# SketchyScene/SketchySceneColorization

Hardware: AMD Instinct MI355X
Metric: train images/sec (192x192, gen+disc fwd+bwd) (higher is better)
Workload: dtype fp32 (bf16x6 split on the bf16 MFMA, fp32 accumulate; filter gradients and few-channel layers on the exact-fp32 MFMA); 1 GPU; Foreground_Instance_Colorization Pix2Pix GAN train step (D-step + G-step, TF-Adam), 192x192, batch 32 per GPU; global_batch=32, parallelism=dp1, ranks_observed_by_allreduce=1, launcher=in-process, block_type=Pix2Pix, launch=hipGraph replay

## Files before the change

### include/sketchycolor_hip.h

```cpp
#ifndef SKETCHYCOLOR_HIP_H
#define SKETCHYCOLOR_HIP_H

#include <stdint.h>

#ifdef __cplusplus
extern "C" {
#endif

#define SSC_ACT_NONE 0
#define SSC_ACT_RELU 1
#define SSC_ACT_LRELU 2
#define SSC_ACT_TANH 3
#define SSC_ACT_PRELU 5
#define SSC_ACT_MIU 4

typedef struct ssc_gview {
    const float* s0;
    const float* s1;
    const float* ab0;
    const float* ab1;
    int32_t C0, C1;
    int32_t H, W;
    int32_t act;
    int32_t act1;
// ... 80 lines not shown
int ssc_conv_forward_bn(const ssc_conv_desc* d, float* ws, int64_t ws_bytes, const float* scale, const float* offset,
                        float eps, float* ab, float* stats, void* stream);
int ssc_head1_forward_supported(const ssc_conv_desc* d);
int ssc_head1_forward(const ssc_conv_desc* d, float* ws, int64_t ws_bytes, void* stream);
int ssc_head1_dgrad_supported(const ssc_conv_desc* d);
int ssc_head1_dgrad(const ssc_conv_desc* d, void* stream);
int ssc_head1_wgrad_supported(const ssc_wgrad_desc* d);
int ssc_head1_wgrad(const ssc_wgrad_desc* d, float* ws, int64_t ws_bytes, void* stream);
int ssc_head1_dgrad_bn_backward(const ssc_conv_desc* d, const float* x, const float* ab, const float* stats, int act,
                                const float* rowb, float rowb_scale, float* dx, float* dscale, float* doffset, float* ws,
                                int64_t ws_bytes, void* stream);
int ssc_bn_bwd_finalize(const float* partial, int nblk, int C, int64_t M, float* coef, float* dscale, float* doffset,
                        void* stream);
int ssc_conv_narrow_supported(const ssc_conv_desc* d);
int ssc_conv_narrow_forward(const ssc_conv_desc* d, void* stream);
int ssc_conv_pw1x1_supported(const ssc_conv_desc* d);
int ssc_conv_c3x3_supported(const ssc_conv_desc* d);
int ssc_conv_s2n16_supported(const ssc_conv_desc* d);
int ssc_conv_tr4n16_supported(const ssc_conv_desc* d);
int ssc_conv_fewchan7_supported(const ssc_conv_desc* d);
int ssc_conv_tr4_tiny_supported(const ssc_conv_desc* d);
int ssc_conv_fewchan_supported(const ssc_conv_desc* d);
int ssc_conv_forward_kernel_name(const ssc_conv_desc* d, char* buf, int len);
int ssc_conv_wgrad_kernel_name(const ssc_wgrad_desc* d, char* buf, int len);
int ssc_conv_forward_plan(const ssc_conv_desc* d, int64_t ws_bytes, int* out5);
int ssc_conv_wgrad_plan(const ssc_wgrad_desc* d, int64_t ws_bytes, int* out4);
int ssc_conv_wgrad128_plan(const ssc_wgrad_desc* d, int64_t ws_bytes, int* out7);
int ssc_conv_bf_plan(const ssc_conv_desc* d, int64_t ws_bytes, int* out10);

int ssc_nchw_to_nhwc(const float* src, float* dst, int N, int C, int HW, int ldc, int coff, void* stream);
// ... 229 lines not shown
```

### sketchyscenecolorization_amd/build.py

```python
import os
import subprocess
import sys

HERE = os.path.dirname(os.path.abspath(__file__))
ROOT = os.path.dirname(HERE)
CSRC = os.path.join(HERE, 'csrc')
LIB_DIR = os.path.join(HERE, 'lib')
LIB_PATH = os.path.join(LIB_DIR, 'libsketchycolor_hip.so')
EXTRA_FLAGS = {'igemm.hip': ['-Xclang', '-target-feature', '-Xclang', '-load-store-opt']} if os.environ.get('SSC_NO_LSOPT') == '1' else {}
NO_PACKED_FP32 = {'narrow.hip': []}
VGPR_FORM = ['-mllvm', '-amdgpu-mfma-vgpr-form=1']
LAST_BUILD = None
SOURCES = ['igemm.hip', 'igemm_bf16.hip', 'wgrad128.hip', 'wgrad128_bf16.hip', 'wgn16.hip', 'narrow.hip', 'head1.hip', 'fewchan.hip', 'fewchan7.hip', 'pw1x1.hip', 'c3x3.hip', 's2n16.hip', 'tr4tiny.hip', 'tr4n16.hip', 'elementwise.hip', 'text_lstm.hip', 'losses_optim.hip', 'mru_ops.hip', 'bg_io.hip', 'bg_scene.hip', 'fg_scene.hip', 'metrics.hip', 'matching.hip', 'match_eval.hip', 'match_train.hip']


def _hipcc():
    for c in (os.environ.get('HIPCC'), '/opt/rocm/bin/hipcc', 'hipcc'):
        if c and (os.path.isabs(c) and os.path.exists(c) or not os.path.isabs(c)):
            return c
    return 'hipcc'


HASH_MARKER = b'SSC_CSRC_HASH='


def tree_hash(csrc=None, header=None):
    import hashlib
    csrc = csrc or CSRC
# ... 33 lines not shown
    import hashlib
    objs = []
    procs = []
    hdrs = b''
    for hp in sorted(os.path.join(CSRC, f) for f in os.listdir(CSRC) if f.endswith('.h')) + [os.path.join(ROOT, 'include', 'sketchycolor_hip.h')]:
        with open(hp, 'rb') as fh:
            hdrs += fh.read()
    for s in SOURCES:
        src = os.path.join(CSRC, s)
        if not os.path.exists(src):
            continue
        obj = os.path.join(LIB_DIR, s.replace('.hip', '.o'))
        cmd = [_hipcc(), '--offload-arch=gfx950', '-O3', '-std=c++17', '-fPIC', '-I' + os.path.join(ROOT, 'include'),
               '-Wno-unused-value', '-Wno-unused-function'] + NO_PACKED_FP32.get(s, ['-fno-slp-vectorize']) + \
              os.environ.get('SSC_EXTRA_HIPCC_FLAGS', '').split() + \
              EXTRA_FLAGS.get(s, []) + (VGPR_FORM if s in ('igemm_bf16.hip', 'wgrad128_bf16.hip') else []) + (['-DSSC_CSRC_HASH="%s"' % th] if s == 'elementwise.hip' else []) + ['-c', src, '-o', obj]
        objs.append(obj)
        with open(src, 'rb') as fh:
            key = hashlib.sha256(fh.read() + b'\0' + hdrs + b'\0' + ' '.join(cmd).encode()).hexdigest()
        kf = obj + '.key'
        if not force and os.path.exists(obj) and os.path.exists(kf) and open(kf).read() == key:
            continue
        if verbose:
            print(' '.join(cmd), flush=True)
        procs.append((subprocess.Popen(cmd), cmd, kf, key))
    for p, cmd, kf, key in procs:
        if p.wait() != 0:
            raise RuntimeError('hipcc failed: ' + ' '.join(cmd))
        with open(kf, 'w') as fh:
            fh.write(key)
    cmd = [_hipcc(), '--offload-arch=gfx950', '-shared', '-fPIC', '-o', LIB_PATH] + objs
# ... 10 lines not shown
```

### sketchyscenecolorization_amd/csrc/igemm.hip

```cpp
#include <hip/hip_runtime.h>
#include <stdint.h>
#include <stdio.h>
#include <stdlib.h>
#include "sketchycolor_hip.h"
#include "igemm_util.h"
#include "igemm_epilogue.h"
#include "host_util.h"

extern "C" int ssc_conv_wgrad128_supported(const ssc_wgrad_desc* dp);
extern "C" int ssc_conv_wgrad128(const ssc_wgrad_desc* dp, float* ws, int64_t ws_bytes, void* stream);
int ssc_conv_wgrad128_bf_selected(const ssc_wgrad_desc* dp);
extern "C" int ssc_conv_wgn16_supported(const ssc_wgrad_desc* dp);
int ssc_conv_wgn16(const ssc_wgrad_desc* dp, float* ws, int64_t ws_bytes, void* stream);
int ssc_conv_wgn16_fits(const ssc_wgrad_desc* dp, int64_t ws_bytes);
int ssc_conv_narrow_forward_ws(const ssc_conv_desc* dp, float* ws, int64_t ws_bytes, void* stream, int* csplit_out);
int ssc_conv_fewchan_forward(const ssc_conv_desc* dp, int num_cu, void* stream);
extern "C" int ssc_conv_pw1x1_supported(const ssc_conv_desc* dp);
int ssc_conv_pw1x1_walkers(const ssc_conv_desc* dp);
int ssc_conv_pw1x1_forward(const ssc_conv_desc* dp, float* stat, void* stream);
extern "C" int ssc_conv_tr4n16_supported(const ssc_conv_desc* dp);
int ssc_conv_tr4n16_rows(const ssc_conv_desc* dp);
int ssc_conv_tr4n16_forward(const ssc_conv_desc* dp, float* stat, void* stream);
extern "C" int ssc_conv_fewchan7_supported(const ssc_conv_desc* dp);
int ssc_conv_fewchan7_walkers(const ssc_conv_desc* dp);
// ... 1457 lines not shown
            if ((double)t128 < plan_const("SSC_PLAN_BF_HK_MIN", 0.5) * 2.0 * num_cu()) {
                return plan_launch(cfgs, 5, allowed_bf, M, d.Nstore, d.nphase, nkt, (long)d.NB * d.OH * d.OW * d.ldc, ws_bytes,
                                   have_ws, can_ts, plan_const("SSC_PLAN_BF_SCALE", 0.45));
            }
            cfgs[0].res = 2;
            cfgs[0].penalty = plan_const("SSC_PLAN_BF_HK", 0.78);
            if (!fwd_is_ut(d)) cfgs[0].penalty *= (double)((d.x.C0 + 15) / 16) / (double)(2 * ((d.x.C0 + 31) / 32));
        }
        return plan_launch(cfgs, 5, allowed_bf, M, d.Nstore, d.nphase, nkt, (long)d.NB * d.OH * d.OW * d.ldc, ws_bytes,
                           have_ws, can_ts, plan_const("SSC_PLAN_BF_SCALE", 0.45));
    }
    return plan_launch(FWD_CFGS, 5, allowed, M, d.Nstore, d.nphase, nkt, (long)d.NB * d.OH * d.OW * d.ldc, ws_bytes,
                       have_ws, can_ts);
}

static void copy_name(const char* src, char* dst, int len) {
    int i = 0;
    for (; i < len - 1 && src[i]; ++i) dst[i] = src[i];
    if (len > 0) dst[i] = 0;
}

extern "C" int ssc_conv_forward_kernel_name(const ssc_conv_desc* dp, char* buf, int len) {
    if (ssc_head1_forward_supported(dp) || ssc_head1_dgrad_supported(dp)) {
        copy_name(ssc_head1_dgrad_supported(dp) ? "head1_dgrad" : "head1_fwd", buf, len);
        return 0;
    }
    if (ssc_conv_narrow_supported(dp)) {
        copy_name(dp->nphase == 4 ? "narrow_fwd<transposed>" : "narrow_fwd<conv>", buf, len);
        return 0;
    }
    if (ssc_conv_fewchan_supported(dp)) {
        copy_name(dp->x.C0 == 8 ? "conv_fewchan<8>" : "conv_fewchan<4>", buf, len);
        return 0;
    }
    if (ssc_conv_pw1x1_supported(dp)) {
        copy_name("conv_pw1x1", buf, len);
        return 0;
    }
    if (ssc_conv_c3x3_supported(dp)) {
// ... 39 lines not shown
                                   const float* offset, float eps, float* ab, float* stats, void* stream) {
    ssc_conv_desc d = *dp;
    d.stat_partial = nullptr;
    d.sb_x = nullptr;
    d.sb2_x = nullptr;
    d.stat_mode = 0;
    const long M = (long)d.NB * d.PH * d.PW;
    const long Mall = M * d.nphase;
    static int off = -1;
    if (off < 0) {
        const char* e = ssc_dev_getenv("SSC_FUSE_STATS");
        off = (e != nullptr && e[0] == '0') ? 1 : 0;
    }
    bool fused = false;
    int64_t ws_conv = ws_bytes;
    const bool earlier = ssc_head1_forward_supported(dp) || ssc_head1_dgrad_supported(dp) || ssc_conv_narrow_supported(dp) ||
                         ssc_conv_fewchan_supported(dp);
    if (!off && !earlier && ws != nullptr && d.Nstore == d.ldc &&
        (ssc_conv_pw1x1_supported(&d) || ssc_conv_c3x3_supported(&d) || ssc_conv_s2n16_supported(&d) ||
         ssc_conv_tr4_tiny_supported(&d) || ssc_conv_fewchan7_supported(&d) || ssc_conv_tr4n16_supported(&d))) {
        const int nblk = ssc_conv_pw1x1_supported(&d) ? ssc_conv_pw1x1_walkers(&d)
                         : (ssc_conv_c3x3_supported(&d) ? ssc_conv_c3x3_walkers(&d)
                            : (ssc_conv_s2n16_supported(&d) ? ssc_conv_s2n16_walkers(&d)
                               : (ssc_conv_tr4_tiny_supported(&d) ? ssc_conv_tr4_tiny_blocks(&d)
                                  : (ssc_conv_fewchan7_supported(&d) ? ssc_conv_fewchan7_walkers(&d) : ssc_conv_tr4n16_rows(&d)))));
        const int64_t need = (int64_t)nblk * 2 * d.Nstore * 4;
        if (need <= ws_bytes) {
            d.stat_partial = ws;
            const int rc = ssc_conv_forward(&d, ws, ws_bytes, stream);
            if (rc != 0) return rc;
            return ssc_bn_finalize(d.stat_partial, nblk, d.Nstore, Mall, scale, offset, eps, ab, stats, stream);
        }
    }
    const bool streaming = ssc_conv_pw1x1_supported(&d) || ssc_conv_c3x3_supported(&d) || ssc_conv_s2n16_supported(&d) ||
                           ssc_conv_tr4_tiny_supported(&d) || ssc_conv_fewchan7_supported(&d) ||
                           ssc_conv_tr4n16_supported(&d);
    if (!off && !streaming && ws != nullptr && !ssc_conv_narrow_supported(dp) && !ssc_conv_fewchan_supported(dp) && d.epi == 0 &&
        !d.accumulate && d.Nstore == d.ldc && ((d.Nstore & 3) == 0) && ((reinterpret_cast<unsigned long>(d.out) & 15) == 0) &&
        (fwd_is_ut(d) || fwd_is_utg(d) || (d.bmode == 0 && fwd_is_rowtap(d)))) {
        const Plan p = plan_fwd(d, ws_bytes, true);
        if (p.cfg >= 0 && p.splitk == 1) {
            const long mt = (M + FWD_CFGS[p.cfg].BM - 1) / FWD_CFGS[p.cfg].BM;
            const int64_t need = (int64_t)mt * d.nphase * 2 * d.Nstore * 4;
            const int64_t reserve = (need + 255) & ~(int64_t)255;
            if (reserve * 4 <= ws_bytes) {
                ws_conv = (ws_bytes - reserve) & ~(int64_t)255;
                const Plan p2 = plan_fwd(d, ws_conv, true);
                if (p2.cfg == p.cfg && p2.splitk == 1) {
                    d.stat_partial = reinterpret_cast<float*>(reinterpret_cast<char*>(ws) + ws_conv);
                    fused = true;
                    const int rc = ssc_conv_forward(&d, ws, ws_conv, stream);
                    if (rc != 0) return rc;
                    return ssc_bn_finalize(d.stat_partial, (int)(mt * d.nphase), d.Nstore, Mall, scale, offset, eps, ab, stats,
                                           stream);
                }
            }
        }
    }
    if (!off && !streaming && ws != nullptr && !ssc_conv_narrow_supported(dp) && !ssc_conv_fewchan_supported(dp) && slab_stats_ok(d) &&
        !(ssc_head1_forward_supported(dp) || ssc_head1_dgrad_supported(dp))) {
        const Plan p = plan_fwd(d, ws_bytes, true);
        if (p.cfg >= 0 && p.splitk > 1 && p.ts_s <= 1) {
            const int nblk = slab_stats_blocks(Mall, d.ldc);
            const int64_t reserve = (((int64_t)nblk * 2 * d.Nstore * 4) + 255) & ~(int64_t)255;
            ws_conv = (ws_bytes - reserve) & ~(int64_t)255;
            const Plan p2 = plan_fwd(d, ws_conv, true);
            if (ws_conv > 0 && p2.cfg == p.cfg && p2.splitk == p.splitk && p2.ts_s <= 1) {
                d.stat_partial = reinterpret_cast<float*>(reinterpret_cast<char*>(ws) + ws_conv);
                const int rc = ssc_conv_forward(&d, ws, ws_conv, stream);
                if (rc != 0) return rc;
                return ssc_bn_finalize(d.stat_partial, nblk, d.Nstore, Mall, scale, offset, eps, ab, stats, stream);
            }
            d.stat_partial = nullptr;
        }
    }
    (void)fused;
    {
        static int dbg = -1;
        if (dbg < 0) {
            const char* e = ssc_dev_getenv("SSC_DEBUG_BNPATH");
            dbg = (e != nullptr && e[0] == '1') ? 1 : 0;
        }
        if (dbg) {
            const Plan p = plan_fwd(d, ws_bytes, ws != nullptr);
            fprintf(stderr, "bnpath separate: M=%ld N=%d K=%d ut=%d utg=%d narrow=%d fewchan=%d cfg=%d splitk=%d epi=%d acc=%d\n", M * d.nphase,
                    d.Nstore, d.TH * d.TW * (d.x.C0 + d.x.C1), (int)fwd_is_ut(d), (int)fwd_is_utg(d), ssc_conv_narrow_supported(dp),
                    ssc_conv_fewchan_supported(dp), p.cfg, p.splitk, d.epi, d.accumulate);
        }
    }
    const int rc = ssc_conv_forward(&d, ws, ws_bytes, stream);
    if (rc != 0) return rc;
    return ssc_bn_stats(d.out, Mall, d.Nstore, d.ldc, scale, offset, eps, ab, stats, ws, ws_bytes, stream);
}

extern "C" int ssc_conv_forward_bnbwd(const ssc_conv_desc* dp, float* ws, int64_t ws_bytes, const float* x, int ldx,
                                      const float* ab, const float* stats, int act, float* partial, int64_t partial_bytes,
                                      int* nrows, void* stream) {
    ssc_conv_desc d = *dp;
    d.stat_partial = nullptr;
    d.sb_x = nullptr;
    d.sb2_x = nullptr;
    d.stat_mode = 0;
    *nrows = 0;
    const long M = (long)d.NB * d.PH * d.PW;
    static int off = -1;
    if (off < 0) {
        const char* e = ssc_dev_getenv("SSC_FUSE_BNBWD");
        off = (e != nullptr && e[0] == '0') ? 1 : 0;
    }
    const bool earlier = ssc_head1_forward_supported(dp) || ssc_head1_dgrad_supported(dp) || ssc_conv_narrow_supported(dp) ||
                         ssc_conv_fewchan_supported(dp);
    if (!off && !earlier && partial != nullptr && x != nullptr && ab != nullptr && stats != nullptr && d.Nstore == d.ldc &&
        (ssc_conv_c3x3_supported(&d) || ssc_conv_s2n16_supported(&d))) {
        const int nblk = ssc_conv_c3x3_supported(&d) ? ssc_conv_c3x3_walkers(&d) : ssc_conv_s2n16_walkers(&d);
        if ((int64_t)nblk * 2 * d.Nstore * 4 <= partial_bytes) {
            d.stat_partial = partial;
            d.sb_x = x; d.sb_ldx = ldx; d.sb_ab = ab; d.sb_stats = stats; d.sb_act = act;
            *nrows = nblk;
            return ssc_conv_forward(&d, ws, ws_bytes, stream);
        }
    }
    if (!off && ws != nullptr && partial != nullptr && x != nullptr && ab != nullptr && stats != nullptr &&
        !ssc_conv_c3x3_supported(&d) && !ssc_conv_s2n16_supported(&d) && !ssc_conv_narrow_supported(dp) && !ssc_conv_fewchan_supported(dp) && d.epi == 0 && !d.accumulate &&
        d.bias == nullptr && d.Nstore == d.ldc &&
        d.Nn == d.Nstore && ((d.Nstore & 3) == 0) && ((ldx & 3) == 0) && ((reinterpret_cast<unsigned long>(d.out) & 15) == 0) &&
        ((reinterpret_cast<unsigned long>(x) & 15) == 0) &&
        (fwd_is_ut(d) || fwd_is_utg(d) || (d.bmode == 0 && fwd_is_rowtap(d)))) {
        const Plan p = plan_fwd(d, ws_bytes, true);
        if (p.cfg >= 0 && p.splitk == 1) {
            const long mt = (M + FWD_CFGS[p.cfg].BM - 1) / FWD_CFGS[p.cfg].BM;
            if ((int64_t)mt * d.nphase * 2 * d.Nstore * 4 <= partial_bytes) {
                d.stat_partial = partial;
                d.sb_x = x; d.sb_ldx = ldx; d.sb_ab = ab; d.sb_stats = stats; d.sb_act = act;
                *nrows = (int)(mt * d.nphase);
            }
        }
    }
    return ssc_conv_forward(&d, ws, ws_bytes, stream);
// ... 4 lines not shown
extern "C" int ssc_minmax_finalize(const float* part, int nsplit, int N, int C, float* mnmx, void* stream);

extern "C" int ssc_conv_forward_minmax(const ssc_conv_desc* dp, float* ws, int64_t ws_bytes, float* mnmx, void* stream) {
    ssc_conv_desc d = *dp;
    d.stat_partial = nullptr;
    d.sb_x = nullptr;
    d.sb2_x = nullptr;
    d.stat_mode = 0;
    const long P = (long)d.PH * d.PW;
    const long M = (long)d.NB * P;
    static int off = -1;
    if (off < 0) {
        const char* e = ssc_dev_getenv("SSC_FUSE_MINMAX");
        off = (e != nullptr && e[0] == '0') ? 1 : 0;
    }
    if (!off && ws != nullptr && d.nphase == 1 && !ssc_conv_narrow_supported(dp) && !ssc_conv_fewchan_supported(dp) &&
        (d.epi == 0 || d.epi == 2) && !d.accumulate && d.Nstore == d.ldc && d.Nn == d.Nstore && ((d.Nstore & 3) == 0) &&
        ((reinterpret_cast<unsigned long>(d.out) & 15) == 0) && (fwd_is_ut(d) || fwd_is_utg(d))) {
        const Plan p = plan_fwd(d, ws_bytes, true);
        if (p.cfg >= 0 && p.splitk == 1 && (P % FWD_CFGS[p.cfg].BM) == 0) {
            const long mt = M / FWD_CFGS[p.cfg].BM;
            const int64_t need = (int64_t)mt * 2 * d.Nstore * 4;
            if (need * 4 <= ws_bytes) {
                const int64_t ws_conv = (ws_bytes - need) & ~(int64_t)255;
                const Plan p2 = plan_fwd(d, ws_conv, true);
                if (p2.cfg == p.cfg && p2.splitk == 1) {
                    d.stat_partial = reinterpret_cast<float*>(reinterpret_cast<char*>(ws) + ws_conv);
                    d.stat_mode = 1;
                    const int rc = ssc_conv_forward(&d, ws, ws_conv, stream);
                    if (rc != 0) return rc;
                    return ssc_minmax_finalize(d.stat_partial, (int)(P / FWD_CFGS[p.cfg].BM), d.NB, d.Nstore, mnmx, stream);
// ... 11 lines not shown
    ssc_conv_desc d = *dp;
    d.stat_partial = nullptr;
    d.sb_x = nullptr;
    d.sb2_x = nullptr;
    d.stat_mode = 0;
    *nrows = 0;
    const long M = (long)d.NB * d.PH * d.PW;
    static int off = -1;
    if (off < 0) {
        const char* e = ssc_dev_getenv("SSC_FUSE_BNBWD");
        off = (e != nullptr && e[0] == '0') ? 1 : 0;
    }
    const int C1 = d.Nstore - C0;
    if (!off && ws != nullptr && s0 != nullptr && s1 != nullptr && s0->x && s1->x && s0->ab && s1->ab && s0->stats && s1->stats &&
        s0->partial && s1->partial && C0 > 0 && C1 > 0 && (C0 % 128) == 0 && (C1 & 3) == 0 &&
        !ssc_conv_narrow_supported(dp) && !ssc_conv_fewchan_supported(dp) && d.epi == 0 && !d.accumulate &&
        d.bias == nullptr && d.Nstore == d.ldc && d.Nn == d.Nstore && ((s0->ldx | s1->ldx) & 3) == 0 &&
        ((reinterpret_cast<unsigned long>(d.out) | reinterpret_cast<unsigned long>(s0->x) |
          reinterpret_cast<unsigned long>(s1->x)) & 15) == 0 &&
        (fwd_is_ut(d) || fwd_is_utg(d))) {
        const Plan p = plan_fwd(d, ws_bytes, true);
        if (p.cfg >= 0 && p.splitk == 1 && FWD_CFGS[p.cfg].BN <= 128) {
            const long mt = (M + FWD_CFGS[p.cfg].BM - 1) / FWD_CFGS[p.cfg].BM;
            if ((int64_t)mt * d.nphase * 2 * C0 * 4 <= s0->partial_bytes && (int64_t)mt * d.nphase * 2 * C1 * 4 <= s1->partial_bytes) {
                d.stat_partial = s0->partial;
                d.sb_x = s0->x; d.sb_ldx = s0->ldx; d.sb_ab = s0->ab; d.sb_stats = s0->stats; d.sb_act = s0->act;
                d.stat_partial2 = s1->partial; d.sb2_col0 = C0;
                d.sb2_x = s1->x; d.sb2_ldx = s1->ldx; d.sb2_ab = s1->ab; d.sb2_stats = s1->stats; d.sb2_act = s1->act;
                *nrows = (int)(mt * d.nphase);
            }
        }
    }
    return ssc_conv_forward(&d, ws, ws_bytes, stream);
}

extern "C" int ssc_sk_configure(int timeout_ms, int test_withhold) {
    const unsigned long long ticks = (unsigned long long)(timeout_ms > 0 ? timeout_ms : 20000) * 100000ull;
    const unsigned cfg[4] = {(unsigned)(ticks & 0xffffffffu), (unsigned)(ticks >> 32), test_withhold ? 1u : 0u, 0u};
    const int rc = ssc_sk_configure_bf(cfg);
    if (rc != 0) return rc;
    return (int)hipMemcpyToSymbol(HIP_SYMBOL(g_sk_cfg), cfg, sizeof(cfg), 0, hipMemcpyHostToDevice);
}

extern "C" int ssc_conv_forward_plan(const ssc_conv_desc* dp, int64_t ws_bytes, int* out5) {
    if (ssc_conv_narrow_supported(dp) || ssc_conv_fewchan_supported(dp)) {
        out5[0] = -1; out5[1] = 1; out5[2] = 0; out5[3] = 1; out5[4] = 0;
        return 0;
    }
    const Plan p = plan_fwd(*dp, ws_bytes, true);
    out5[0] = p.cfg; out5[1] = p.splitk; out5[2] = (int)p.ts_full; out5[3] = p.ts_s; out5[4] = (int)(p.cost / 1000.0);
    return 0;
}

static int fwd_desc_error(const ssc_conv_desc& d) {
    if ((d.x.C0 & 3) || (d.x.C1 & 3) || d.Nstore < d.Nn || d.Nstore > d.ldc) return -1;
    if (d.nphase != 1 && d.nphase != 4) return -2;
    if (d.nphase == 4 && (d.TH != 2 || d.TW != 2 || d.KH != 4 || d.KW != 4 || d.kstep != -2 || d.out_stride != 2 ||
                          d.in_stride != 1))
        return -3;
    return 0;
}
enum { FWD_TILED = 0, FWD_HEAD1, FWD_HEAD1_DGRAD, FWD_NARROW, FWD_FEWCHAN, FWD_PW1X1, FWD_C3X3, FWD_S2N16, FWD_TR4_TINY, FWD_FEWCHAN7,
       FWD_TR4N16 };
static int fwd_early_kernel(const ssc_conv_desc* dp, bool have_ws, int64_t ws_bytes) {
    const ssc_conv_desc& d = *dp;
    if (have_ws && ssc_head1_forward_supported(dp) && (int64_t)d.NB * d.x.H * d.x.W * 16 * 4 <= ws_bytes) return FWD_HEAD1;
    if (ssc_head1_dgrad_supported(dp)) return FWD_HEAD1_DGRAD;
    if (ssc_conv_narrow_supported(dp)) return FWD_NARROW;
    if (ssc_conv_fewchan_supported(dp)) return FWD_FEWCHAN;
    if (ssc_conv_pw1x1_supported(dp)) return FWD_PW1X1;
    if (ssc_conv_c3x3_supported(dp)) return FWD_C3X3;
    if (ssc_conv_s2n16_supported(dp)) return FWD_S2N16;
    if (ssc_conv_tr4_tiny_supported(dp)) return FWD_TR4_TINY;
    if (ssc_conv_fewchan7_supported(dp)) return FWD_FEWCHAN7;
    if (ssc_conv_tr4n16_supported(dp)) return FWD_TR4N16;
    return FWD_TILED;
}
static bool fwd_bf_plain(const ssc_conv_desc& d) {
    const bool plain0 = d.x.ab0 == nullptr && d.x.act == SSC_ACT_NONE;
    const bool plain1 = d.x.C1 == 0 || (d.x.ab1 == nullptr && (d.x.act1 >= 0 ? d.x.act1 : d.x.act) == SSC_ACT_NONE);
    return plain0 && plain1;
}
// ... 5 lines not shown
    if (err != 0) return err;
    if (fwd_early_kernel(dp, have_ws, ws_bytes) != FWD_TILED || !fwd_is_bf(d)) return -10;
    const Plan p = plan_fwd(d, ws_bytes, have_ws);
    if (p.cfg < 0) return -4;
    return ssc_conv_bf_form(p.cfg, fwd_bf_plain(d), d, p.splitk, have_ws, p.ts_full, p.ts_s, ws_bytes, xcd_order(), out10);
}

extern "C" int ssc_conv_forward(const ssc_conv_desc* dp, float* ws, int64_t ws_bytes, void* stream) {
    const ssc_conv_desc& d = *dp;
    hipStream_t st = (hipStream_t)stream;
    const int err = fwd_desc_error(d);
    if (err != 0) return err;
    switch (fwd_early_kernel(dp, ws != nullptr, ws_bytes)) {
        case FWD_HEAD1: return ssc_head1_forward(dp, ws, ws_bytes, stream);
        case FWD_HEAD1_DGRAD: return ssc_head1_dgrad(dp, stream);
        case FWD_NARROW: {
            int csplit = 1;
            const int rc = ssc_conv_narrow_forward_ws(dp, ws, ws_bytes, stream, &csplit);
            if (rc != 0 || csplit == 1) return rc;
            const long out_count = (long)d.NB * d.OH * d.OW * d.ldc;
            hipLaunchKernelGGL(slab_reduce_kernel, dim3((unsigned)((out_count + 255) / 256)), dim3(256), 0, st, ws, out_count,
                               csplit, d.out, out_count, d.ldc, d.Nn, d.Nstore, d.bias, d.epi, d.accumulate);
            return (int)hipGetLastError();
        }
        case FWD_FEWCHAN: return ssc_conv_fewchan_forward(dp, num_cu(), stream);
        case FWD_PW1X1: return ssc_conv_pw1x1_forward(dp, d.stat_partial, stream);
        case FWD_C3X3: return ssc_conv_c3x3_forward(dp, d.stat_partial, stream);
        case FWD_S2N16: return ssc_conv_s2n16_forward(dp, d.stat_partial, stream);
        case FWD_TR4_TINY: return ssc_conv_tr4_tiny_forward(dp, d.stat_partial, stream);
        case FWD_FEWCHAN7: return ssc_conv_fewchan7_forward(dp, d.stat_partial, stream);
// ... 194 lines not shown
```

### sketchyscenecolorization_amd/hip.py

```python
import ctypes as C
import os

import torch

_HERE = os.path.dirname(os.path.abspath(__file__))
LIB_PATH = os.environ.get('SSC_LIB_PATH') or os.path.join(_HERE, 'lib', 'libsketchycolor_hip.so')

ACT_PRELU = 5
ACT_NONE, ACT_RELU, ACT_LRELU, ACT_TANH, ACT_MIU = 0, 1, 2, 3, 4


class GView(C.Structure):
    _fields_ = [('s0', C.c_void_p), ('s1', C.c_void_p), ('ab0', C.c_void_p), ('ab1', C.c_void_p),
                ('C0', C.c_int32), ('C1', C.c_int32), ('H', C.c_int32), ('W', C.c_int32),
                ('act', C.c_int32), ('act1', C.c_int32)]


class ConvDesc(C.Structure):
    _fields_ = [('x', GView), ('w', C.c_void_p), ('bias', C.c_void_p), ('out', C.c_void_p),
                ('NB', C.c_int32), ('PH', C.c_int32), ('PW', C.c_int32),
                ('TH', C.c_int32), ('TW', C.c_int32), ('in_stride', C.c_int32),
                ('ioff_y', C.c_int32), ('ioff_x', C.c_int32), ('nphase', C.c_int32),
                ('ky0', C.c_int32), ('kx0', C.c_int32), ('kstep', C.c_int32),
                ('KH', C.c_int32), ('KW', C.c_int32), ('wC0', C.c_int32), ('wC1', C.c_int32),
# ... 108 lines not shown
    'ssc_bn_act_backward_pre': [_P, _L, _I, _I, _P, _P, _P, _I, _I, _P, _I, _I, _I, _P, _I, _P, _P, _P, _I, _P, _F, _I, _P,
                                _L, _P],
    'ssc_head1_forward_supported': [C.POINTER(ConvDesc)],
    'ssc_head1_forward': [C.POINTER(ConvDesc), _P, _L, _P],
    'ssc_head1_dgrad_supported': [C.POINTER(ConvDesc)],
    'ssc_head1_dgrad': [C.POINTER(ConvDesc), _P],
    'ssc_head1_wgrad_supported': [C.POINTER(WgradDesc)],
    'ssc_head1_wgrad': [C.POINTER(WgradDesc), _P, _L, _P],
    'ssc_head1_dgrad_bn_backward': [C.POINTER(ConvDesc), _P, _P, _P, _I, _P, _F, _P, _P, _P, _P, _L, _P],
    'ssc_bn_bwd_finalize': [_P, _I, _I, _L, _P, _P, _P, _P],
    'ssc_block_out_backward': [_P, _P, _L, _I, _I, _P, _P, _P, _P, _P, _P, _P, _P, _P, _P, _P, _P, _P, _P, _P, _L, _P],
    'ssc_bn_bwd_sums': [C.POINTER(BnApplyJob), _P, _I, _P, _P, _P, _P, _L, _P],
    'ssc_bn_bwd_apply': [C.POINTER(BnApplyJob), _P],
    'ssc_conv_narrow_supported': [C.POINTER(ConvDesc)],
    'ssc_conv_narrow_forward': [C.POINTER(ConvDesc), _P],
    'ssc_conv_fewchan_supported': [C.POINTER(ConvDesc)],
    'ssc_conv_pw1x1_supported': [C.POINTER(ConvDesc)],
    'ssc_conv_c3x3_supported': [C.POINTER(ConvDesc)],
    'ssc_conv_s2n16_supported': [C.POINTER(ConvDesc)],
    'ssc_conv_tr4n16_supported': [C.POINTER(ConvDesc)],
    'ssc_conv_fewchan7_supported': [C.POINTER(ConvDesc)],
    'ssc_conv_tr4_tiny_supported': [C.POINTER(ConvDesc)],
    'ssc_conv_forward_kernel_name': [C.POINTER(ConvDesc), C.c_char_p, _I],
    'ssc_conv_wgrad_kernel_name': [C.POINTER(WgradDesc), C.c_char_p, _I],
    'ssc_conv_forward_plan': [C.POINTER(ConvDesc), _L, C.POINTER(C.c_int)],
    'ssc_conv_wgrad_plan': [C.POINTER(WgradDesc), _L, C.POINTER(C.c_int)],
    'ssc_conv_wgrad128_plan': [C.POINTER(WgradDesc), _L, C.POINTER(C.c_int)],
    'ssc_conv_bf_plan': [C.POINTER(ConvDesc), _L, C.POINTER(C.c_int)],
    'ssc_sk_configure': [_I, _I],
    'ssc_nchw_to_nhwc': [_P, _P, _I, _I, _I, _I, _I, _P],
# ... 1450 lines not shown
```

Baseline: 2482 images/sec.

## Add bf16x6 MFMA kernel for narrow-output 4x4 stride-2 transposed convolutions

Adds a new kernel for transposed 4x4 stride-2 convolutions with at most four output channels, typically the generator's final RGB layer. It computes all 16 taps per input pixel as a small GEMM on the bf16 MFMA using a three-way bf16 split (six products) to keep near-fp32 accuracy. The per-tap results are staged in LDS and summed into the four output phases, with the next tile's input prefetched while MFMAs run. It takes priority over the existing narrow kernel. It adds LDS pressure, recomputes the halo rows at tile edges, and changes the rounding behaviour compared with the previous fp32 path.

Measured after the change: 2512 images/sec (median of 6 runs). 1.01x the previous value.

```diff
diff --git a/include/sketchycolor_hip.h b/include/sketchycolor_hip.h
--- a/include/sketchycolor_hip.h
+++ b/include/sketchycolor_hip.h
@@ -118,6 +118,8 @@
                         void* stream);
 int ssc_conv_narrow_supported(const ssc_conv_desc* d);
 int ssc_conv_narrow_forward(const ssc_conv_desc* d, void* stream);
+int ssc_conv_tr4bf_supported(const ssc_conv_desc* d);
+int ssc_conv_tr4bf_forward(const ssc_conv_desc* d, void* stream);
 int ssc_conv_pw1x1_supported(const ssc_conv_desc* d);
 int ssc_conv_c3x3_supported(const ssc_conv_desc* d);
 int ssc_conv_s2n16_supported(const ssc_conv_desc* d);
diff --git a/sketchyscenecolorization_amd/build.py b/sketchyscenecolorization_amd/build.py
--- a/sketchyscenecolorization_amd/build.py
+++ b/sketchyscenecolorization_amd/build.py
@@ -11,7 +11,7 @@
 NO_PACKED_FP32 = {'narrow.hip': []}
 VGPR_FORM = ['-mllvm', '-amdgpu-mfma-vgpr-form=1']
 LAST_BUILD = None
-SOURCES = ['igemm.hip', 'igemm_bf16.hip', 'wgrad128.hip', 'wgrad128_bf16.hip', 'wgn16.hip', 'narrow.hip', 'head1.hip', 'fewchan.hip', 'fewchan7.hip', 'pw1x1.hip', 'c3x3.hip', 's2n16.hip', 'tr4tiny.hip', 'tr4n16.hip', 'elementwise.hip', 'text_lstm.hip', 'losses_optim.hip', 'mru_ops.hip', 'bg_io.hip', 'bg_scene.hip', 'fg_scene.hip', 'metrics.hip', 'matching.hip', 'match_eval.hip', 'match_train.hip']
+SOURCES = ['igemm.hip', 'igemm_bf16.hip', 'wgrad128.hip', 'wgrad128_bf16.hip', 'wgn16.hip', 'narrow.hip', 'tr4bf.hip', 'head1.hip', 'fewchan.hip', 'fewchan7.hip', 'pw1x1.hip', 'c3x3.hip', 's2n16.hip', 'tr4tiny.hip', 'tr4n16.hip', 'elementwise.hip', 'text_lstm.hip', 'losses_optim.hip', 'mru_ops.hip', 'bg_io.hip', 'bg_scene.hip', 'fg_scene.hip', 'metrics.hip', 'matching.hip', 'match_eval.hip', 'match_train.hip']
 
 
 def _hipcc():
@@ -75,7 +75,7 @@
         cmd = [_hipcc(), '--offload-arch=gfx950', '-O3', '-std=c++17', '-fPIC', '-I' + os.path.join(ROOT, 'include'),
                '-Wno-unused-value', '-Wno-unused-function'] + NO_PACKED_FP32.get(s, ['-fno-slp-vectorize']) + \
               os.environ.get('SSC_EXTRA_HIPCC_FLAGS', '').split() + \
-              EXTRA_FLAGS.get(s, []) + (VGPR_FORM if s in ('igemm_bf16.hip', 'wgrad128_bf16.hip') else []) + (['-DSSC_CSRC_HASH="%s"' % th] if s == 'elementwise.hip' else []) + ['-c', src, '-o', obj]
+              EXTRA_FLAGS.get(s, []) + (VGPR_FORM if s in ('igemm_bf16.hip', 'wgrad128_bf16.hip', 'tr4bf.hip') else []) + (['-DSSC_CSRC_HASH="%s"' % th] if s == 'elementwise.hip' else []) + ['-c', src, '-o', obj]
         objs.append(obj)
         with open(src, 'rb') as fh:
             key = hashlib.sha256(fh.read() + b'\0' + hdrs + b'\0' + ' '.join(cmd).encode()).hexdigest()
diff --git a/sketchyscenecolorization_amd/csrc/igemm.hip b/sketchyscenecolorization_amd/csrc/igemm.hip
--- a/sketchyscenecolorization_amd/csrc/igemm.hip
+++ b/sketchyscenecolorization_amd/csrc/igemm.hip
@@ -1495,6 +1495,8 @@
                        have_ws, can_ts);
 }
 
+static bool fwd_is_narrow(const ssc_conv_desc* dp) { return ssc_conv_narrow_supported(dp) || ssc_conv_tr4bf_supported(dp); }
+
 static void copy_name(const char* src, char* dst, int len) {
     int i = 0;
     for (; i < len - 1 && src[i]; ++i) dst[i] = src[i];
@@ -1504,6 +1506,10 @@
 extern "C" int ssc_conv_forward_kernel_name(const ssc_conv_desc* dp, char* buf, int len) {
     if (ssc_head1_forward_supported(dp) || ssc_head1_dgrad_supported(dp)) {
         copy_name(ssc_head1_dgrad_supported(dp) ? "head1_dgrad" : "head1_fwd", buf, len);
+        return 0;
+    }
+    if (ssc_conv_tr4bf_supported(dp)) {
+        copy_name("narrow_bf16x6<transposed>", buf, len);
         return 0;
     }
     if (ssc_conv_narrow_supported(dp)) {
@@ -1573,7 +1579,7 @@
     }
     bool fused = false;
     int64_t ws_conv = ws_bytes;
-    const bool earlier = ssc_head1_forward_supported(dp) || ssc_head1_dgrad_supported(dp) || ssc_conv_narrow_supported(dp) ||
+    const bool earlier = ssc_head1_forward_supported(dp) || ssc_head1_dgrad_supported(dp) || fwd_is_narrow(dp) ||
                          ssc_conv_fewchan_supported(dp);
     if (!off && !earlier && ws != nullptr && d.Nstore == d.ldc &&
         (ssc_conv_pw1x1_supported(&d) || ssc_conv_c3x3_supported(&d) || ssc_conv_s2n16_supported(&d) ||
@@ -1594,7 +1600,7 @@
     const bool streaming = ssc_conv_pw1x1_supported(&d) || ssc_conv_c3x3_supported(&d) || ssc_conv_s2n16_supported(&d) ||
                            ssc_conv_tr4_tiny_supported(&d) || ssc_conv_fewchan7_supported(&d) ||
                            ssc_conv_tr4n16_supported(&d);
-    if (!off && !streaming && ws != nullptr && !ssc_conv_narrow_supported(dp) && !ssc_conv_fewchan_supported(dp) && d.epi == 0 &&
+    if (!off && !streaming && ws != nullptr && !fwd_is_narrow(dp) && !ssc_conv_fewchan_supported(dp) && d.epi == 0 &&
         !d.accumulate && d.Nstore == d.ldc && ((d.Nstore & 3) == 0) && ((reinterpret_cast<unsigned long>(d.out) & 15) == 0) &&
         (fwd_is_ut(d) || fwd_is_utg(d) || (d.bmode == 0 && fwd_is_rowtap(d)))) {
         const Plan p = plan_fwd(d, ws_bytes, true);
@@ -1616,7 +1622,7 @@
             }
         }
     }
-    if (!off && !streaming && ws != nullptr && !ssc_conv_narrow_supported(dp) && !ssc_conv_fewchan_supported(dp) && slab_stats_ok(d) &&
+    if (!off && !streaming && ws != nullptr && !fwd_is_narrow(dp) && !ssc_conv_fewchan_supported(dp) && slab_stats_ok(d) &&
         !(ssc_head1_forward_supported(dp) || ssc_head1_dgrad_supported(dp))) {
         const Plan p = plan_fwd(d, ws_bytes, true);
         if (p.cfg >= 0 && p.splitk > 1 && p.ts_s <= 1) {
@@ -1643,7 +1649,7 @@
         if (dbg) {
             const Plan p = plan_fwd(d, ws_bytes, ws != nullptr);
             fprintf(stderr, "bnpath separate: M=%ld N=%d K=%d ut=%d utg=%d narrow=%d fewchan=%d cfg=%d splitk=%d epi=%d acc=%d\n", M * d.nphase,
-                    d.Nstore, d.TH * d.TW * (d.x.C0 + d.x.C1), (int)fwd_is_ut(d), (int)fwd_is_utg(d), ssc_conv_narrow_supported(dp),
+                    d.Nstore, d.TH * d.TW * (d.x.C0 + d.x.C1), (int)fwd_is_ut(d), (int)fwd_is_utg(d), (int)fwd_is_narrow(dp),
                     ssc_conv_fewchan_supported(dp), p.cfg, p.splitk, d.epi, d.accumulate);
         }
     }
@@ -1667,7 +1673,7 @@
         const char* e = ssc_dev_getenv("SSC_FUSE_BNBWD");
         off = (e != nullptr && e[0] == '0') ? 1 : 0;
     }
-    const bool earlier = ssc_head1_forward_supported(dp) || ssc_head1_dgrad_supported(dp) || ssc_conv_narrow_supported(dp) ||
+    const bool earlier = ssc_head1_forward_supported(dp) || ssc_head1_dgrad_supported(dp) || fwd_is_narrow(dp) ||
                          ssc_conv_fewchan_supported(dp);
     if (!off && !earlier && partial != nullptr && x != nullptr && ab != nullptr && stats != nullptr && d.Nstore == d.ldc &&
         (ssc_conv_c3x3_supported(&d) || ssc_conv_s2n16_supported(&d))) {
@@ -1680,7 +1686,7 @@
         }
     }
     if (!off && ws != nullptr && partial != nullptr && x != nullptr && ab != nullptr && stats != nullptr &&
-        !ssc_conv_c3x3_supported(&d) && !ssc_conv_s2n16_supported(&d) && !ssc_conv_narrow_supported(dp) && !ssc_conv_fewchan_supported(dp) && d.epi == 0 && !d.accumulate &&
+        !ssc_conv_c3x3_supported(&d) && !ssc_conv_s2n16_supported(&d) && !fwd_is_narrow(dp) && !ssc_conv_fewchan_supported(dp) && d.epi == 0 && !d.accumulate &&
         d.bias == nullptr && d.Nstore == d.ldc &&
         d.Nn == d.Nstore && ((d.Nstore & 3) == 0) && ((ldx & 3) == 0) && ((reinterpret_cast<unsigned long>(d.out) & 15) == 0) &&
         ((reinterpret_cast<unsigned long>(x) & 15) == 0) &&
@@ -1715,7 +1721,7 @@
         const char* e = ssc_dev_getenv("SSC_FUSE_MINMAX");
         off = (e != nullptr && e[0] == '0') ? 1 : 0;
     }
-    if (!off && ws != nullptr && d.nphase == 1 && !ssc_conv_narrow_supported(dp) && !ssc_conv_fewchan_supported(dp) &&
+    if (!off && ws != nullptr && d.nphase == 1 && !fwd_is_narrow(dp) && !ssc_conv_fewchan_supported(dp) &&
         (d.epi == 0 || d.epi == 2) && !d.accumulate && d.Nstore == d.ldc && d.Nn == d.Nstore && ((d.Nstore & 3) == 0) &&
         ((reinterpret_cast<unsigned long>(d.out) & 15) == 0) && (fwd_is_ut(d) || fwd_is_utg(d))) {
         const Plan p = plan_fwd(d, ws_bytes, true);
@@ -1757,7 +1763,7 @@
     const int C1 = d.Nstore - C0;
     if (!off && ws != nullptr && s0 != nullptr && s1 != nullptr && s0->x && s1->x && s0->ab && s1->ab && s0->stats && s1->stats &&
         s0->partial && s1->partial && C0 > 0 && C1 > 0 && (C0 % 128) == 0 && (C1 & 3) == 0 &&
-        !ssc_conv_narrow_supported(dp) && !ssc_conv_fewchan_supported(dp) && d.epi == 0 && !d.accumulate &&
+        !fwd_is_narrow(dp) && !ssc_conv_fewchan_supported(dp) && d.epi == 0 && !d.accumulate &&
         d.bias == nullptr && d.Nstore == d.ldc && d.Nn == d.Nstore && ((s0->ldx | s1->ldx) & 3) == 0 &&
         ((reinterpret_cast<unsigned long>(d.out) | reinterpret_cast<unsigned long>(s0->x) |
           reinterpret_cast<unsigned long>(s1->x)) & 15) == 0 &&
@@ -1786,7 +1792,7 @@
 }
 
 extern "C" int ssc_conv_forward_plan(const ssc_conv_desc* dp, int64_t ws_bytes, int* out5) {
-    if (ssc_conv_narrow_supported(dp) || ssc_conv_fewchan_supported(dp)) {
+    if (fwd_is_narrow(dp) || ssc_conv_fewchan_supported(dp)) {
         out5[0] = -1; out5[1] = 1; out5[2] = 0; out5[3] = 1; out5[4] = 0;
         return 0;
     }
@@ -1804,11 +1810,12 @@
     return 0;
 }
 enum { FWD_TILED = 0, FWD_HEAD1, FWD_HEAD1_DGRAD, FWD_NARROW, FWD_FEWCHAN, FWD_PW1X1, FWD_C3X3, FWD_S2N16, FWD_TR4_TINY, FWD_FEWCHAN7,
-       FWD_TR4N16 };
+       FWD_TR4N16, FWD_TR4BF };
 static int fwd_early_kernel(const ssc_conv_desc* dp, bool have_ws, int64_t ws_bytes) {
     const ssc_conv_desc& d = *dp;
     if (have_ws && ssc_head1_forward_supported(dp) && (int64_t)d.NB * d.x.H * d.x.W * 16 * 4 <= ws_bytes) return FWD_HEAD1;
     if (ssc_head1_dgrad_supported(dp)) return FWD_HEAD1_DGRAD;
+    if (ssc_conv_tr4bf_supported(dp)) return FWD_TR4BF;
     if (ssc_conv_narrow_supported(dp)) return FWD_NARROW;
     if (ssc_conv_fewchan_supported(dp)) return FWD_FEWCHAN;
     if (ssc_conv_pw1x1_supported(dp)) return FWD_PW1X1;
@@ -1844,6 +1851,7 @@
     switch (fwd_early_kernel(dp, ws != nullptr, ws_bytes)) {
         case FWD_HEAD1: return ssc_head1_forward(dp, ws, ws_bytes, stream);
         case FWD_HEAD1_DGRAD: return ssc_head1_dgrad(dp, stream);
+        case FWD_TR4BF: return ssc_conv_tr4bf_forward(dp, stream);
         case FWD_NARROW: {
             int csplit = 1;
             const int rc = ssc_conv_narrow_forward_ws(dp, ws, ws_bytes, stream, &csplit);
diff --git a/sketchyscenecolorization_amd/csrc/tr4bf.hip b/sketchyscenecolorization_amd/csrc/tr4bf.hip
--- /dev/null
+++ b/sketchyscenecolorization_amd/csrc/tr4bf.hip
@@ -0,0 +1,289 @@
+#include <hip/hip_runtime.h>
+#include <stdint.h>
+#include <stdlib.h>
+#include "sketchycolor_hip.h"
+#include "igemm_util.h"
+#include "igemm_epilogue.h"
+#include "host_util.h"
+
+#define TB_R 8
+#define TB_W 16
+#define TB_PIX (TB_R * TB_W)
+#define TB_LDS_MAX (64 * 1024)
+
+typedef short bf16x8 __attribute__((ext_vector_type(8)));
+typedef __bf16 bf16x2_t __attribute__((ext_vector_type(2)));
+typedef unsigned u32x4_t __attribute__((ext_vector_type(4)));
+
+__device__ __forceinline__ unsigned tb_cvt_pk_bf16(float a, float b) {
+    const f32x2_t v = {a, b};
+    return __builtin_bit_cast(unsigned, __builtin_convertvector(v, bf16x2_t));
+}
+__device__ __forceinline__ void tb_split3_pair(float x0, float x1, unsigned& h, unsigned& m, unsigned& l) {
+    h = tb_cvt_pk_bf16(x0, x1);
+    const float r0 = x0 - __uint_as_float(h << 16), r1 = x1 - __uint_as_float(h & 0xffff0000u);
+    m = tb_cvt_pk_bf16(r0, r1);
+    const float s0 = r0 - __uint_as_float(m << 16), s1 = r1 - __uint_as_float(m & 0xffff0000u);
+    l = tb_cvt_pk_bf16(s0, s1);
+}
+__device__ __forceinline__ void tb_split8(const float4& u, const float4& v, bf16x8& h, bf16x8& m, bf16x8& l) {
+    unsigned hh[4], mm[4], ll[4];
+    tb_split3_pair(u.x, u.y, hh[0], mm[0], ll[0]);
+    tb_split3_pair(u.z, u.w, hh[1], mm[1], ll[1]);
+    tb_split3_pair(v.x, v.y, hh[2], mm[2], ll[2]);
+    tb_split3_pair(v.z, v.w, hh[3], mm[3], ll[3]);
+    h = __builtin_bit_cast(bf16x8, (u32x4_t){hh[0], hh[1], hh[2], hh[3]});
+    m = __builtin_bit_cast(bf16x8, (u32x4_t){mm[0], mm[1], mm[2], mm[3]});
+    l = __builtin_bit_cast(bf16x8, (u32x4_t){ll[0], ll[1], ll[2], ll[3]});
+}
+
+static inline size_t tb_lds_bytes(int C, int nout) {
+    const size_t NC = 16 * (size_t)nout;
+    return (size_t)6 * C * NC + (size_t)TB_PIX * NC * 4 + (size_t)8 * C;
+}
+
+template <int NOUT>
+__global__ __launch_bounds__(256) __attribute__((amdgpu_waves_per_eu(4))) void tr4bf_kernel(const ssc_conv_desc d, int tiles, int tiles_x, int tiles_y) {
+    constexpr int NC = 16 * NOUT, NB = (NC + 31) / 32;
+    extern __shared__ __attribute__((aligned(16))) unsigned char tb_smem[];
+    const int C = d.x.C0 + d.x.C1, S = C >> 4;
+    u32x4_t* const wf = reinterpret_cast<u32x4_t*>(tb_smem);
+    float* const T = reinterpret_cast<float*>(tb_smem + (size_t)6 * C * NC);
+    float* const abl = T + TB_PIX * NC;
+    const int tid = threadIdx.x, lane = tid & 63, wave = tid >> 6;
+    const int l31 = lane & 31, lhi = lane >> 5;
+    const int H = d.x.H, W = d.x.W;
+
+    {
+        const long w_ts = (long)d.wC0 * d.wC1;
+        const long w_ns = (d.bmode == 0) ? 0 : (long)d.wC1;
+        const float* wb = d.w + ((d.bmode == 0) ? (long)d.n_off : (long)d.n_off * d.wC1);
+        for (int it = tid; it < S * 2 * NC; it += 256) {
+            const int col = it % NC, r = it / NC;
+            const int lh = r & 1, s = r >> 1;
+            const int tap = col / NOUT, c = col - tap * NOUT;
+            const bool v = c < d.Nn;
+            const float* wp = v ? wb + tap * w_ts + c * w_ns + 16 * s + 4 * lh : d.w;
+            float4 u0 = *reinterpret_cast<const float4*>(wp), u1 = *reinterpret_cast<const float4*>(wp + (v ? 8 : 0));
+            if (!v) u0 = u1 = make_float4(0.f, 0.f, 0.f, 0.f);
+            bf16x8 h, m, l;
+            tb_split8(u0, u1, h, m, l);
+            wf[((s * 2 + lh) * 3 + 0) * NC + col] = __builtin_bit_cast(u32x4_t, h);
+            wf[((s * 2 + lh) * 3 + 1) * NC + col] = __builtin_bit_cast(u32x4_t, m);
+            wf[((s * 2 + lh) * 3 + 2) * NC + col] = __builtin_bit_cast(u32x4_t, l);
+        }
+        for (int c = tid; c < C; c += 256) {
+            const bool first = c < d.x.C0;
+            const float* abp = first ? d.x.ab0 : d.x.ab1;
+            const int cc = first ? c : c - d.x.C0, cs = first ? d.x.C0 : d.x.C1;
+            abl[(c >> 2) * 8 + (c & 3)] = abp != nullptr ? abp[cc] : 1.f;
+            abl[(c >> 2) * 8 + 4 + (c & 3)] = abp != nullptr ? abp[cs + cc] : 0.f;
+        }
+    }
+    const float slope0 = act_slope(d.x.act), slope1 = act_slope(d.x.act1 >= 0 ? d.x.act1 : d.x.act);
+
+    const int prow = (wave * 32 + l31) / TB_W, pcol = (wave * 32 + l31) % TB_W;
+    struct TilePos { int n, i0, j0; };
+    auto tile_pos = [&](int tile) {
+        TilePos t;
+        const int txi = tile % tiles_x, r = tile / tiles_x;
+        const int tyi = r % tiles_y;
+        t.n = r / tiles_y;
+        t.i0 = tyi * (TB_R - 1) - 1;
+        t.j0 = txi * (TB_W - 1) - 1;
+        return t;
+    };
+    auto tile_poff = [&](const TilePos& t) {
+        const int iy = t.i0 + prow, ix = t.j0 + pcol;
+        const bool ok = ((unsigned)iy < (unsigned)H) & ((unsigned)ix < (unsigned)W);
+        return ok ? (t.n * H + iy) * W + ix : -1;
+    };
+    float4 rv[2][2];
+    auto load_half = [&](int poff, int cb, int j) {
+        const bool first = cb < d.x.C0;
+        const char* src = reinterpret_cast<const char*>(first ? d.x.s0 : d.x.s1);
+        const unsigned cs = first ? d.x.C0 : d.x.C1;
+        const unsigned cc = first ? cb : cb - d.x.C0;
+        const unsigned off = ((poff >= 0 ? (unsigned)poff * cs : 0u) + cc + 16 * j + 4 * lhi) * 4u;
+#pragma unroll
+        for (int q = 0; q < 2; ++q) rv[j][q] = *reinterpret_cast<const float4*>(src + (size_t)(off + 32u * q));
+    };
+
+    const int G = gridDim.x;
+    int tile = blockIdx.x;
+    TilePos tp = tile_pos(tile < tiles ? tile : 0);
+    int poff = tile < tiles ? tile_poff(tp) : -1;
+    if (tile < tiles) {
+        load_half(poff, 0, 0);
+        load_half(poff, 0, 1);
+    }
+    __syncthreads();
+
+    for (; tile < tiles; tile += G) {
+        const int next = tile + G;
+        const TilePos tpn = tile_pos(next < tiles ? next : 0);
+        const int poff_n = next < tiles ? tile_poff(tpn) : -1;
+        f32x16 acc[NB], accc[NB];
+#pragma unroll
+        for (int j = 0; j < NB; ++j)
+#pragma unroll
+            for (int r = 0; r < 16; ++r) { acc[j][r] = 0.f; accc[j][r] = 0.f; }
+
+        for (int cb = 0; cb < C; cb += 32) {
+            const float slope = cb < d.x.C0 ? slope0 : slope1;
+            const bool ok = poff >= 0;
+#pragma unroll
+            for (int j = 0; j < 2; ++j) {
+                float4 x[2];
+#pragma unroll
+                for (int q = 0; q < 2; ++q) {
+                    const int c0 = cb + 16 * j + 8 * q + 4 * lhi;
+                    const float4 a = *reinterpret_cast<const float4*>(abl + 2 * c0);
+                    const float4 b = *reinterpret_cast<const float4*>(abl + 2 * c0 + 4);
+                    const float4 t = xform4(rv[j][q], a, b, slope, 1.f);
+                    x[q] = ok ? t : make_float4(0.f, 0.f, 0.f, 0.f);
+                }
+                bf16x8 ah, am, al;
+                tb_split8(x[0], x[1], ah, am, al);
+                {
+                    const bool more = cb + 32 < C;
+                    load_half(more ? poff : poff_n, more ? cb + 32 : 0, j);
+                }
+                __builtin_amdgcn_sched_barrier(0);
+                const int s = (cb >> 4) + j;
+                int col[NB];
+#pragma unroll
+                for (int nb = 0; nb < NB; ++nb) col[nb] = (nb * 32 + l31 < NC) ? nb * 32 + l31 : NC - 1;
+                auto bop = [&](int plane, int nb) { return __builtin_bit_cast(bf16x8, wf[((s * 2 + lhi) * 3 + plane) * NC + col[nb]]); };
+                bf16x8 bh[NB], bx[NB];
+#pragma unroll
+                for (int nb = 0; nb < NB; ++nb) bh[nb] = bop(0, nb);
+#pragma unroll
+                for (int nb = 0; nb < NB; ++nb) accc[nb] = __builtin_amdgcn_mfma_f32_32x32x16_bf16(al, bh[nb], accc[nb], 0, 0, 0);
+#pragma unroll
+                for (int nb = 0; nb < NB; ++nb) bx[nb] = bop(2, nb);
+#pragma unroll
+                for (int nb = 0; nb < NB; ++nb) accc[nb] = __builtin_amdgcn_mfma_f32_32x32x16_bf16(ah, bx[nb], accc[nb], 0, 0, 0);
+#pragma unroll
+                for (int nb = 0; nb < NB; ++nb) bx[nb] = bop(1, nb);
+#pragma unroll
+                for (int nb = 0; nb < NB; ++nb) accc[nb] = __builtin_amdgcn_mfma_f32_32x32x16_bf16(am, bx[nb], accc[nb], 0, 0, 0);
+#pragma unroll
+                for (int nb = 0; nb < NB; ++nb) accc[nb] = __builtin_amdgcn_mfma_f32_32x32x16_bf16(am, bh[nb], accc[nb], 0, 0, 0);
+#pragma unroll
+                for (int nb = 0; nb < NB; ++nb) accc[nb] = __builtin_amdgcn_mfma_f32_32x32x16_bf16(ah, bx[nb], accc[nb], 0, 0, 0);
+#pragma unroll
+                for (int nb = 0; nb < NB; ++nb) acc[nb] = __builtin_amdgcn_mfma_f32_32x32x16_bf16(ah, bh[nb], acc[nb], 0, 0, 0);
+                __builtin_amdgcn_sched_barrier(0);
+            }
+        }
+
+#pragma unroll
+        for (int nb = 0; nb < NB; ++nb) {
+            const int col = nb * 32 + l31;
+            if (col < NC) {
+#pragma unroll
+                for (int r = 0; r < 16; ++r) {
+                    const int pix = wave * 32 + (r & 3) + 8 * (r >> 2) + 4 * lhi;
+                    T[pix * NC + col] = acc[nb][r] + accc[nb][r];
+                }
+            }
+        }
+        __syncthreads();
+
+        constexpr int OXT = 2 * (TB_W - 1), OYT = 2 * (TB_R - 1);
+        for (int it = tid; it < OXT * OYT; it += 256) {
+            const int oyl = it / OXT, oxl = it - oyl * OXT;
+            const int oy = 2 * tp.i0 + 1 + oyl, ox = 2 * tp.j0 + 1 + oxl;
+            if ((unsigned)oy >= (unsigned)d.OH || (unsigned)ox >= (unsigned)d.OW) continue;
+            const int py = oy >> 1, px = ox >> 1;
+            const FwdPhase ph = fwd_phase(d, (oy & 1) * 2 + (ox & 1));
+            float v[NOUT];
+#pragma unroll
+            for (int t = 0; t < 4; ++t) {
+                const int ty = t >> 1, tx = t & 1;
+                const int ry = py + ph.ioff_y + ty - tp.i0, rx = px + ph.ioff_x + tx - tp.j0;
+                const int tap = (ph.ky0 + ty * d.kstep) * d.KW + ph.kx0 + tx * d.kstep;
+                const float* tq = T + (ry * TB_W + rx) * NC + tap * NOUT;
+#pragma unroll
+                for (int n = 0; n < NOUT; ++n) v[n] = (t == 0) ? tq[n] : v[n] + tq[n];
+            }
+            float* o = d.out + (((long)tp.n * d.OH + oy) * d.OW + ox) * d.ldc;
+#pragma unroll
+            for (int n = 0; n < 4; ++n) {
+                if (n >= d.Nstore) break;
+                float r = 0.f;
+                if (n < NOUT && n < d.Nn) {
+                    r = v[n < NOUT ? n : 0];
+                    if (d.bias != nullptr) r += d.bias[n];
+                    if (d.epi == 1) r = tanhf(r);
+                    else if (d.epi == 2) r = fmaxf(r, 0.2f * r);
+                    if (d.accumulate) r += o[n];
+                }
+                o[n] = r;
+            }
+        }
+        __syncthreads();
+        tp = tpn;
+        poff = poff_n;
+    }
+}
+
+static bool tb_on() {
+    static int on = -1;
+    if (on < 0) {
+        const char* e = ssc_dev_getenv("SSC_TR4BF");
+        const char* a = getenv("SSC_ARITH");
+        on = ((e != nullptr && e[0] == '0') || (a != nullptr && (a[0] == 'f' || a[0] == 'F'))) ? 0 : 1;
+    }
+    return on != 0;
+}
+
+extern "C" int ssc_conv_tr4bf_supported(const ssc_conv_desc* dp) {
+    const ssc_conv_desc& d = *dp;
+    if (!tb_on()) return 0;
+    if (d.nphase != 4 || d.TH != 2 || d.TW != 2 || d.KH != 4 || d.KW != 4 || d.out_stride != 2 || d.in_stride != 1 || d.ky0 != 0 ||
+        d.kx0 != 0 || d.kstep != -2 || d.ioff_y != 0 || d.ioff_x != 0 || d.ooff_y != 0 || d.ooff_x != 0)
+        return 0;
+    if (d.Nn < 1 || d.Nn > 4 || d.Nstore > 4 || d.Nstore < d.Nn || d.Nstore > d.ldc) return 0;
+    const int C = d.x.C0 + d.x.C1;
+    if (C < 32 || (C % 32) != 0 || (d.x.C0 % 32) != 0 || d.k_real != C) return 0;
+    if (tb_lds_bytes(C, d.Nn) > TB_LDS_MAX) return 0;
+    const bool kcontig = (d.bmode == 1) ? (d.wC1 % 4 == 0 && d.wC1 >= C && d.n_off >= 0 && d.n_off + d.Nn <= d.wC0)
+                                        : (d.wC1 == 1 && d.Nn == 1 && d.n_off == 0 && d.wC0 >= C && d.wC0 % 4 == 0);
+    if (!kcontig || (reinterpret_cast<uintptr_t>(d.w) & 15) != 0) return 0;
+    if (d.x.H != d.PH || d.x.W != d.PW || d.OH != 2 * d.PH || d.OW != 2 * d.PW) return 0;
+    if ((reinterpret_cast<uintptr_t>(d.x.s0) & 15) != 0 || (d.x.C1 > 0 && (reinterpret_cast<uintptr_t>(d.x.s1) & 15) != 0)) return 0;
+    if (d.x.act != SSC_ACT_NONE && d.x.act != SSC_ACT_RELU && d.x.act != SSC_ACT_LRELU) return 0;
+    if (d.x.act1 > SSC_ACT_LRELU) return 0;
+    if (d.epi < 0 || d.epi > 2) return 0;
+    if (d.stat_partial != nullptr || d.sb_x != nullptr || d.sb2_x != nullptr || d.stat_mode != 0) return 0;
+    if ((long)d.NB * d.x.H * d.x.W >= 0x7fffffffL) return 0;
+    if ((long)d.NB * d.x.H * d.x.W * (d.x.C0 > d.x.C1 ? d.x.C0 : d.x.C1) * 4 > 0xffffffffL) return 0;
+    return 1;
+}
+
+template <int NOUT>
+static int tb_launch(const ssc_conv_desc& d, hipStream_t st) {
+    static unsigned long long attr_done = 0;
+    const int arc = ssc_set_max_lds(reinterpret_cast<const void*>(&tr4bf_kernel<NOUT>), TB_LDS_MAX, &attr_done);
+    if (arc != 0) return arc;
+    const int tiles_y = (d.x.H + 1 + TB_R - 2) / (TB_R - 1), tiles_x = (d.x.W + 1 + TB_W - 2) / (TB_W - 1);
+    const long tiles = (long)d.NB * tiles_y * tiles_x;
+    if (tiles >= 0x7fffffffL) return -5;
+    const long g = 2L * ssc_num_cu();
+    hipLaunchKernelGGL(tr4bf_kernel<NOUT>, dim3((unsigned)(tiles < g ? tiles : g)), dim3(256), tb_lds_bytes(d.x.C0 + d.x.C1, NOUT), st, d,
+                       (int)tiles, tiles_x, tiles_y);
+    return (int)hipGetLastError();
+}
+
+extern "C" int ssc_conv_tr4bf_forward(const ssc_conv_desc* dp, void* stream) {
+    if (!ssc_conv_tr4bf_supported(dp)) return -1;
+    hipStream_t st = (hipStream_t)stream;
+    switch (dp->Nn) {
+        case 1: return tb_launch<1>(*dp, st);
+        case 2: return tb_launch<2>(*dp, st);
+        case 3: return tb_launch<3>(*dp, st);
+        default: return tb_launch<4>(*dp, st);
+    }
+}
diff --git a/sketchyscenecolorization_amd/hip.py b/sketchyscenecolorization_amd/hip.py
--- a/sketchyscenecolorization_amd/hip.py
+++ b/sketchyscenecolorization_amd/hip.py
@@ -146,6 +146,8 @@
     'ssc_bn_bwd_apply': [C.POINTER(BnApplyJob), _P],
     'ssc_conv_narrow_supported': [C.POINTER(ConvDesc)],
     'ssc_conv_narrow_forward': [C.POINTER(ConvDesc), _P],
+    'ssc_conv_tr4bf_supported': [C.POINTER(ConvDesc)],
+    'ssc_conv_tr4bf_forward': [C.POINTER(ConvDesc), _P],
     'ssc_conv_fewchan_supported': [C.POINTER(ConvDesc)],
     'ssc_conv_pw1x1_supported': [C.POINTER(ConvDesc)],
     'ssc_conv_c3x3_supported': [C.POINTER(ConvDesc)],
```
